# nexus-rl/dfd-starter

Hardware: AMD Instinct MI355X
Metric: env steps/sec (whole node) + sec/FD-grad-step, 4096 antithetic perturbations (higher is better)
Workload: dtype f32; 1 GPU; BASELINE config 3: HalfCheetah-shaped synthetic env (obs 17, act 6), MujocoPolicy(17,6) P=6092, 4096 antithetic perturbations per GPU (2048 directions x +/-), T=1000 fixed-length episodes, full FD step (rollout + weights + gradient + DSGD); perturbations_per_gpu=4096, envs_per_perturbation=1, global_perturbations=4096, episode_len=1000, n_params=6092, parallelism=dp1

## Files before the change

### dfd-starter_amd/csrc/fdr_dpp_gen.h

```cpp
#pragma once

namespace fdr {

__device__ __forceinline__ void dpp_dot_32x1(float& a0, float X0, float X1, const float* w) {
  asm volatile(
      "s_nop 1\n\t"
      "v_mul_f32_dpp %0, %1, %3 row_newbcast:0 row_mask:0xf bank_mask:0xf\n\t"
      "v_fmac_f32_dpp %0, %2, %19 row_newbcast:0 row_mask:0xf bank_mask:0xf\n\t"
      "v_fmac_f32_dpp %0, %1, %4 row_newbcast:1 row_mask:0xf bank_mask:0xf\n\t"
      "v_fmac_f32_dpp %0, %2, %20 row_newbcast:1 row_mask:0xf bank_mask:0xf\n\t"
      "v_fmac_f32_dpp %0, %1, %5 row_newbcast:2 row_mask:0xf bank_mask:0xf\n\t"
      "v_fmac_f32_dpp %0, %2, %21 row_newbcast:2 row_mask:0xf bank_mask:0xf\n\t"
      "v_fmac_f32_dpp %0, %1, %6 row_newbcast:3 row_mask:0xf bank_mask:0xf\n\t"
      "v_fmac_f32_dpp %0, %2, %22 row_newbcast:3 row_mask:0xf bank_mask:0xf\n\t"
      "v_fmac_f32_dpp %0, %1, %7 row_newbcast:4 row_mask:0xf bank_mask:0xf\n\t"
      "v_fmac_f32_dpp %0, %2, %23 row_newbcast:4 row_mask:0xf bank_mask:0xf\n\t"
      "v_fmac_f32_dpp %0, %1, %8 row_newbcast:5 row_mask:0xf bank_mask:0xf\n\t"
      "v_fmac_f32_dpp %0, %2, %24 row_newbcast:5 row_mask:0xf bank_mask:0xf\n\t"
      "v_fmac_f32_dpp %0, %1, %9 row_newbcast:6 row_mask:0xf bank_mask:0xf\n\t"
      "v_fmac_f32_dpp %0, %2, %25 row_newbcast:6 row_mask:0xf bank_mask:0xf\n\t"
      "v_fmac_f32_dpp %0, %1, %10 row_newbcast:7 row_mask:0xf bank_mask:0xf\n\t"
      "v_fmac_f32_dpp %0, %2, %26 row_newbcast:7 row_mask:0xf bank_mask:0xf\n\t"
      "v_fmac_f32_dpp %0, %1, %11 row_newbcast:8 row_mask:0xf bank_mask:0xf\n\t"
      "v_fmac_f32_dpp %0, %2, %27 row_newbcast:8 row_mask:0xf bank_mask:0xf\n\t"
      "v_fmac_f32_dpp %0, %1, %12 row_newbcast:9 row_mask:0xf bank_mask:0xf\n\t"
      "v_fmac_f32_dpp %0, %2, %28 row_newbcast:9 row_mask:0xf bank_mask:0xf\n\t"
      "v_fmac_f32_dpp %0, %1, %13 row_newbcast:10 row_mask:0xf bank_mask:0xf\n\t"
      "v_fmac_f32_dpp %0, %2, %29 row_newbcast:10 row_mask:0xf bank_mask:0xf\n\t"
      "v_fmac_f32_dpp %0, %1, %14 row_newbcast:11 row_mask:0xf bank_mask:0xf\n\t"
      "v_fmac_f32_dpp %0, %2, %30 row_newbcast:11 row_mask:0xf bank_mask:0xf\n\t"
      "v_fmac_f32_dpp %0, %1, %15 row_newbcast:12 row_mask:0xf bank_mask:0xf\n\t"
      "v_fmac_f32_dpp %0, %2, %31 row_newbcast:12 row_mask:0xf bank_mask:0xf\n\t"
      "v_fmac_f32_dpp %0, %1, %16 row_newbcast:13 row_mask:0xf bank_mask:0xf\n\t"
      "v_fmac_f32_dpp %0, %2, %32 row_newbcast:13 row_mask:0xf bank_mask:0xf\n\t"
      "v_fmac_f32_dpp %0, %1, %17 row_newbcast:14 row_mask:0xf bank_mask:0xf\n\t"
      "v_fmac_f32_dpp %0, %2, %33 row_newbcast:14 row_mask:0xf bank_mask:0xf\n\t"
      "v_fmac_f32_dpp %0, %1, %18 row_newbcast:15 row_mask:0xf bank_mask:0xf\n\t"
      "v_fmac_f32_dpp %0, %2, %34 row_newbcast:15 row_mask:0xf bank_mask:0xf\n\t"
      : "=&v"(a0)
      : "v"(X0), "v"(X1), "v"(w[0]), "v"(w[1]), "v"(w[2]), "v"(w[3]), "v"(w[4]), "v"(w[5]), "v"(w[6]), "v"(w[7]), "v"(w[8]), "v"(w[9]), "v"(w[10]), "v"(w[11]), "v"(w[12]), "v"(w[13]), "v"(w[14]), "v"(w[15]), "v"(w[16]), "v"(w[17]), "v"(w[18]), "v"(w[19]), "v"(w[20]), "v"(w[21]), "v"(w[22]), "v"(w[23]), "v"(w[24]), "v"(w[25]), "v"(w[26]), "v"(w[27]), "v"(w[28]), "v"(w[29]), "v"(w[30]), "v"(w[31]));
}
__device__ __forceinline__ void dpp_dot_16x4(float& a0, float& a1, float& a2, float& a3, float X0, const float* w) {
  asm volatile(
      "s_nop 1\n\t"
      "v_mul_f32_dpp %0, %4, %5 row_newbcast:0 row_mask:0xf bank_mask:0xf\n\t"
      "v_mul_f32_dpp %1, %4, %6 row_newbcast:1 row_mask:0xf bank_mask:0xf\n\t"
      "v_mul_f32_dpp %2, %4, %7 row_newbcast:2 row_mask:0xf bank_mask:0xf\n\t"
      "v_mul_f32_dpp %3, %4, %8 row_newbcast:3 row_mask:0xf bank_mask:0xf\n\t"
      "v_fmac_f32_dpp %0, %4, %9 row_newbcast:4 row_mask:0xf bank_mask:0xf\n\t"
      "v_fmac_f32_dpp %1, %4, %10 row_newbcast:5 row_mask:0xf bank_mask:0xf\n\t"
      "v_fmac_f32_dpp %2, %4, %11 row_newbcast:6 row_mask:0xf bank_mask:0xf\n\t"
      "v_fmac_f32_dpp %3, %4, %12 row_newbcast:7 row_mask:0xf bank_mask:0xf\n\t"
      "v_fmac_f32_dpp %0, %4, %13 row_newbcast:8 row_mask:0xf bank_mask:0xf\n\t"
      "v_fmac_f32_dpp %1, %4, %14 row_newbcast:9 row_mask:0xf bank_mask:0xf\n\t"
      "v_fmac_f32_dpp %2, %4, %15 row_newbcast:10 row_mask:0xf bank_mask:0xf\n\t"
      "v_fmac_f32_dpp %3, %4, %16 row_newbcast:11 row_mask:0xf bank_mask:0xf\n\t"
      "v_fmac_f32_dpp %0, %4, %17 row_newbcast:12 row_mask:0xf bank_mask:0xf\n\t"
      "v_fmac_f32_dpp %1, %4, %18 row_newbcast:13 row_mask:0xf bank_mask:0xf\n\t"
      "v_fmac_f32_dpp %2, %4, %19 row_newbcast:14 row_mask:0xf bank_mask:0xf\n\t"
      "v_fmac_f32_dpp %3, %4, %20 row_newbcast:15 row_mask:0xf bank_mask:0xf\n\t"
      : "=&v"(a0), "=&v"(a1), "=&v"(a2), "=&v"(a3)
      : "v"(X0), "v"(w[0]), "v"(w[1]), "v"(w[2]), "v"(w[3]), "v"(w[4]), "v"(w[5]), "v"(w[6]), "v"(w[7]), "v"(w[8]), "v"(w[9]), "v"(w[10]), "v"(w[11]), "v"(w[12]), "v"(w[13]), "v"(w[14]), "v"(w[15]));
}
__device__ __forceinline__ void dpp_fma_tail1(float& a0, float X0, const float* w) {
  asm volatile(
      "s_nop 1\n\t"
      "v_fmac_f32_dpp %0, %1, %2 row_newbcast:0 row_mask:0xf bank_mask:0xf\n\t"
      : "+v"(a0)
      : "v"(X0), "v"(w[0]));
}
__device__ __forceinline__ void dpp_fma_tail2(float& a0, float X0, const float* w) {
  asm volatile(
      "s_nop 1\n\t"
      "v_fmac_f32_dpp %0, %1, %2 row_newbcast:0 row_mask:0xf bank_mask:0xf\n\t"
// ... 166 lines not shown
      "v_fmac_f32_dpp %0, %1, %7 row_newbcast:5 row_mask:0xf bank_mask:0xf\n\t"
      "v_fmac_f32_dpp %0, %1, %8 row_newbcast:6 row_mask:0xf bank_mask:0xf\n\t"
      "v_fmac_f32_dpp %0, %1, %9 row_newbcast:7 row_mask:0xf bank_mask:0xf\n\t"
      "v_fmac_f32_dpp %0, %1, %10 row_newbcast:8 row_mask:0xf bank_mask:0xf\n\t"
      "v_fmac_f32_dpp %0, %1, %11 row_newbcast:9 row_mask:0xf bank_mask:0xf\n\t"
      "v_fmac_f32_dpp %0, %1, %12 row_newbcast:10 row_mask:0xf bank_mask:0xf\n\t"
      "v_fmac_f32_dpp %0, %1, %13 row_newbcast:11 row_mask:0xf bank_mask:0xf\n\t"
      "v_fmac_f32_dpp %0, %1, %14 row_newbcast:12 row_mask:0xf bank_mask:0xf\n\t"
      "v_fmac_f32_dpp %0, %1, %15 row_newbcast:13 row_mask:0xf bank_mask:0xf\n\t"
      : "+v"(a0)
      : "v"(X0), "v"(w[0]), "v"(w[1]), "v"(w[2]), "v"(w[3]), "v"(w[4]), "v"(w[5]), "v"(w[6]), "v"(w[7]), "v"(w[8]), "v"(w[9]), "v"(w[10]), "v"(w[11]), "v"(w[12]), "v"(w[13]));
}
__device__ __forceinline__ void dpp_fma_tail15(float& a0, float X0, const float* w) {
  asm volatile(
      "s_nop 1\n\t"
      "v_fmac_f32_dpp %0, %1, %2 row_newbcast:0 row_mask:0xf bank_mask:0xf\n\t"
      "v_fmac_f32_dpp %0, %1, %3 row_newbcast:1 row_mask:0xf bank_mask:0xf\n\t"
      "v_fmac_f32_dpp %0, %1, %4 row_newbcast:2 row_mask:0xf bank_mask:0xf\n\t"
      "v_fmac_f32_dpp %0, %1, %5 row_newbcast:3 row_mask:0xf bank_mask:0xf\n\t"
      "v_fmac_f32_dpp %0, %1, %6 row_newbcast:4 row_mask:0xf bank_mask:0xf\n\t"
      "v_fmac_f32_dpp %0, %1, %7 row_newbcast:5 row_mask:0xf bank_mask:0xf\n\t"
      "v_fmac_f32_dpp %0, %1, %8 row_newbcast:6 row_mask:0xf bank_mask:0xf\n\t"
      "v_fmac_f32_dpp %0, %1, %9 row_newbcast:7 row_mask:0xf bank_mask:0xf\n\t"
      "v_fmac_f32_dpp %0, %1, %10 row_newbcast:8 row_mask:0xf bank_mask:0xf\n\t"
      "v_fmac_f32_dpp %0, %1, %11 row_newbcast:9 row_mask:0xf bank_mask:0xf\n\t"
      "v_fmac_f32_dpp %0, %1, %12 row_newbcast:10 row_mask:0xf bank_mask:0xf\n\t"
      "v_fmac_f32_dpp %0, %1, %13 row_newbcast:11 row_mask:0xf bank_mask:0xf\n\t"
      "v_fmac_f32_dpp %0, %1, %14 row_newbcast:12 row_mask:0xf bank_mask:0xf\n\t"
      "v_fmac_f32_dpp %0, %1, %15 row_newbcast:13 row_mask:0xf bank_mask:0xf\n\t"
      "v_fmac_f32_dpp %0, %1, %16 row_newbcast:14 row_mask:0xf bank_mask:0xf\n\t"
      : "+v"(a0)
      : "v"(X0), "v"(w[0]), "v"(w[1]), "v"(w[2]), "v"(w[3]), "v"(w[4]), "v"(w[5]), "v"(w[6]), "v"(w[7]), "v"(w[8]), "v"(w[9]), "v"(w[10]), "v"(w[11]), "v"(w[12]), "v"(w[13]), "v"(w[14]));
}
}
```

### dfd-starter_amd/csrc/fdr_mlp_pair.h

```cpp
#pragma once
#include "fdr_mlp.h"

namespace fdr {

constexpr int kPairWaves = 2;

__device__ __forceinline__ f2 tanh2_pre(f2 t) {
  const f2 d = f2{__builtin_amdgcn_exp2f(t.x), __builtin_amdgcn_exp2f(t.y)} + f2{1.f, 1.f};
  return pk_fma(f2{-2.f, -2.f}, f2{__builtin_amdgcn_rcpf(d.x), __builtin_amdgcn_rcpf(d.y)}, f2{1.f, 1.f});
}
__device__ __forceinline__ f2 tanh2_fast(f2 x) {
  return tanh2_pre(x * f2{kTanhScale, kTanhScale});
}
constexpr float kPreScale = kTanhScale;
template <bool kPre>
__device__ __forceinline__ f2 tanh2_act(f2 z) {
  if constexpr (kPre) return tanh2_pre(z);
  else return tanh2_fast(z);
}

template <int NIN, int NA, bool DISC>
struct MlpPair {
  using L = Layout<NIN, NA, DISC>;
  static constexpr int NOUT = L::NOUT;
  static constexpr int NX = round4(NIN);
  static_assert(NX <= 32, "pair kernel: policy input wider than 32");
  static constexpr bool kBiasCol = NIN < NX;
  static constexpr bool kW1Lds = NIN > 8;
  static constexpr bool kPre = !DISC;
  static constexpr float kWS = kPre ? kTanhScale : 1.f;
  static constexpr int kW1Chunks = kW1Lds ? NX / 4 : 0;
  static constexpr int kTileF4 = (2 * kW1Chunks + 8) * kWave;
  f2 w1a[kW1Lds ? 1 : NX / 2], w1b[kW1Lds ? 1 : NX / 2];
  float b1a, b1b;
  const float4* tile;
  f2 w2[64];
  float b2a, b2b, b3;
  float a0, c0, a1a, c1a, a1b, c1b, a2a, c2a, a2b, c2b;

  __host__ __device__ static constexpr int head_unit(int rho, int k, int e) {
    return 32 * rho + 8 * (k >> 2) + 4 * e + (k & 3);
  }

// ... 97 lines not shown
      fold(L::BN1W, L::BN1B, NIN, ua, a1a, c1a);
      fold(L::BN1W, L::BN1B, NIN, ub, a1b, c1b);
      fold(L::BN2W, L::BN2B, NIN + kHidden, u2a, a2a, c2a);
      fold(L::BN2W, L::BN2B, NIN + kHidden, u2b, a2b, c2b);
    }
  }

  __device__ __forceinline__ float input_transform(float x) const {
    if constexpr (DISC) {
      return fmaf(x, a0, c0);
    } else {
      return x;
    }
  }

  __device__ __forceinline__ float act1(float z, float av, float cv) const {
    if constexpr (DISC) {
      return fmaf(fmaxf(z, 0.f), av, cv);
    } else {
      return tanh_act<kPre>(z);
    }
  }

  static constexpr bool kTail = kW1Lds && kBiasCol && NX - NIN == 3;
  static constexpr int NQ = kTail ? NX / 4 - 1 : NX / 4;
  static constexpr bool kPk = kW1Lds && kBiasCol;
  static constexpr int kPkPairs = (NIN + 2) / 2;
  struct L1Rows {
    float4 wa[kW1Lds && !kPk ? NQ : 1], wb[kW1Lds && !kPk ? NQ : 1], m[NQ];
    float2 ta, tb;
    float tm;
    float4 wp[kPk ? kPkPairs : 1];
  };
  __device__ __forceinline__ void l1_prefetch(L1Rows& r, const float* mrow) const {
    const float4* m4 = reinterpret_cast<const float4*>(mrow);
#pragma unroll
    for (int q = 0; q < NQ; ++q) {
      if constexpr (kW1Lds && !kPk) {
        r.wa[q] = tile[q * kWave];
        r.wb[q] = tile[(kW1Chunks + q) * kWave];
      }
      r.m[q] = m4[q];
    }
    if constexpr (kPk) {
#pragma unroll
      for (int j = 0; j < kPkPairs; ++j) r.wp[j] = tile[j * kWave];
      if constexpr (kTail) r.tm = mrow[4 * NQ];
    } else if constexpr (kTail) {
      r.ta = *reinterpret_cast<const float2*>(&tile[NQ * kWave]);
      r.tb = *reinterpret_cast<const float2*>(&tile[(kW1Chunks + NQ) * kWave]);
      r.tm = mrow[4 * NQ];
    }
  }

  struct SIn {
    float4 v[NQ];
    float t;
  };
  template <bool kSameInput, class Fill>
  __device__ __forceinline__ f2 layer1_env(const float* xs, const float* ss, const L1Rows& rows, SIn& sin,
                                           Fill&& fill) const {
    const float4* x4 = reinterpret_cast<const float4*>(xs);
    const float4* s4 = reinterpret_cast<const float4*>(ss);
    SIn xin;
#pragma unroll
    for (int q = 0; q < NQ; ++q) {
      xin.v[q] = x4[q];
      sin.v[q] = kSameInput ? xin.v[q] : s4[q];
    }
    xin.t = kTail ? xs[4 * NQ] : 0.f;
    sin.t = kSameInput ? xin.t : (kTail ? ss[4 * NQ] : 0.f);
    fill();
    __builtin_amdgcn_sched_barrier(0);
    return layer1_q(xin, rows);
  }
  __device__ __forceinline__ float env_ms(const SIn& sin, const L1Rows& rows) const {
    f2 am0 = {0.f, 0.f}, am1 = {0.f, 0.f};
#pragma unroll
    for (int q = 0; q < NQ; ++q) {
      const float4 sv = sin.v[q], mv = rows.m[q];
      am0 = pk_fma(f2{mv.x, mv.y}, f2{sv.x, sv.y}, am0);
      am1 = pk_fma(f2{mv.z, mv.w}, f2{sv.z, sv.w}, am1);
    }
    if constexpr (kTail) am1.x = fmaf(rows.tm, sin.t, am1.x);
    const f2 am = am0 + am1;
    return am.x + am.y;
// ... 40 lines not shown
        return f2{act1(h.x, a1a, c1a), act1(h.y, a1b, c1b)};
      } else {
        return tanh2_act<kPre>(h);
      }
    }
#pragma unroll
    for (int q = 0; q < NQ; ++q) {
      const float4 xv = xq(q);
      float4 wa, wb;
      if constexpr (kW1Lds) {
        wa = rows.wa[q];
        wb = rows.wb[q];
      } else {
        wa = float4{w1a[2 * q].x, w1a[2 * q].y, w1a[2 * q + 1].x, w1a[2 * q + 1].y};
        wb = float4{w1b[2 * q].x, w1b[2 * q].y, w1b[2 * q + 1].x, w1b[2 * q + 1].y};
      }
      aa0 = pk_fma(f2{wa.x, wa.y}, f2{xv.x, xv.y}, aa0);
      ab0 = pk_fma(f2{wb.x, wb.y}, f2{xv.x, xv.y}, ab0);
      aa1 = pk_fma(f2{wa.z, wa.w}, f2{xv.z, xv.w}, aa1);
      ab1 = pk_fma(f2{wb.z, wb.w}, f2{xv.z, xv.w}, ab1);
    }
    if constexpr (kTail) {
      aa1 = pk_fma(f2{rows.ta.x, rows.ta.y}, f2{xt, 1.f}, aa1);
      ab1 = pk_fma(f2{rows.tb.x, rows.tb.y}, f2{xt, 1.f}, ab1);
    }
    const f2 ha = aa0 + aa1, hb = ab0 + ab1;
    if constexpr (DISC) {
      return f2{act1(ha.x + ha.y, a1a, c1a), act1(hb.x + hb.y, a1b, c1b)};
    } else {
      return tanh2_act<kPre>(f2{ha.x + ha.y, hb.x + hb.y});
    }
  }

  template <class Mark>
  __device__ __forceinline__ float layers23(f2 h1, float* h1s, int t, Mark&& mark) const {
    const int c4 = t & 3;
    float x[16];
    reinterpret_cast<f2*>(h1s)[t] = h1;
    __builtin_amdgcn_s_setprio(0);
    wave_lds_sync();
    lds_bcast<16>(h1s + 16 * c4, x);
    float w3[32];
#pragma unroll
    for (int m = 0; m < 8; ++m) {
      const float4 w = tile[(2 * kW1Chunks + m) * kWave];
      w3[4 * m] = w.x;
      w3[4 * m + 1] = w.y;
      w3[4 * m + 2] = w.z;
      w3[4 * m + 3] = w.w;
    }
    f2 acc[4];
#pragma unroll
    for (int p = 0; p < 4; ++p)
      acc[p] = pk_fma(w2[p * 16], f2{x[0], x[0]}, (kPre && p == 0) ? f2{b2a, b2b} : f2{0.f, 0.f});
    {
      f2 xp[8];
#pragma unroll
      for (int j = 0; j < 8; ++j) xp[j] = f2{x[2 * j], x[2 * j + 1]};
#define FDR_L2_HI "op_sel:[0,1,0] op_sel_hi:[1,1,1]"
#define FDR_L2_LO "op_sel_hi:[1,0,1]"
      asm(
          "v_pk_fma_f32 %0, %4, %64, %0 " FDR_L2_HI "\n"
          "v_pk_fma_f32 %1, %5, %64, %1 " FDR_L2_HI "\n"
          "v_pk_fma_f32 %2, %6, %64, %2 " FDR_L2_HI "\n"
          "v_pk_fma_f32 %3, %7, %64, %3 " FDR_L2_HI "\n"
          "v_pk_fma_f32 %0, %8, %65, %0 " FDR_L2_LO "\n"
          "v_pk_fma_f32 %1, %9, %65, %1 " FDR_L2_LO "\n"
          "v_pk_fma_f32 %2, %10, %65, %2 " FDR_L2_LO "\n"
// ... 40 lines not shown
          "v_pk_fma_f32 %3, %51, %70, %3 " FDR_L2_LO "\n"
          "v_pk_fma_f32 %0, %52, %70, %0 " FDR_L2_HI "\n"
          "v_pk_fma_f32 %1, %53, %70, %1 " FDR_L2_HI "\n"
          "v_pk_fma_f32 %2, %54, %70, %2 " FDR_L2_HI "\n"
          "v_pk_fma_f32 %3, %55, %70, %3 " FDR_L2_HI "\n"
          "v_pk_fma_f32 %0, %56, %71, %0 " FDR_L2_LO "\n"
          "v_pk_fma_f32 %1, %57, %71, %1 " FDR_L2_LO "\n"
          "v_pk_fma_f32 %2, %58, %71, %2 " FDR_L2_LO "\n"
          "v_pk_fma_f32 %3, %59, %71, %3 " FDR_L2_LO "\n"
          "v_pk_fma_f32 %3, %63, %71, %3 " FDR_L2_HI "\n"
          "v_pk_fma_f32 %2, %62, %71, %2 " FDR_L2_HI "\n"
          "v_pk_fma_f32 %0, %60, %71, %0 " FDR_L2_HI "\n"
          "v_pk_fma_f32 %1, %61, %71, %1 " FDR_L2_HI "\n"
          : "+v"(acc[0]), "+v"(acc[1]), "+v"(acc[2]), "+v"(acc[3])
          : "v"(w2[1]), "v"(w2[17]), "v"(w2[33]), "v"(w2[49]),
            "v"(w2[2]), "v"(w2[18]), "v"(w2[34]), "v"(w2[50]),
            "v"(w2[3]), "v"(w2[19]), "v"(w2[35]), "v"(w2[51]),
            "v"(w2[4]), "v"(w2[20]), "v"(w2[36]), "v"(w2[52]),
            "v"(w2[5]), "v"(w2[21]), "v"(w2[37]), "v"(w2[53]),
            "v"(w2[6]), "v"(w2[22]), "v"(w2[38]), "v"(w2[54]),
            "v"(w2[7]), "v"(w2[23]), "v"(w2[39]), "v"(w2[55]),
            "v"(w2[8]), "v"(w2[24]), "v"(w2[40]), "v"(w2[56]),
            "v"(w2[9]), "v"(w2[25]), "v"(w2[41]), "v"(w2[57]),
            "v"(w2[10]), "v"(w2[26]), "v"(w2[42]), "v"(w2[58]),
            "v"(w2[11]), "v"(w2[27]), "v"(w2[43]), "v"(w2[59]),
            "v"(w2[12]), "v"(w2[28]), "v"(w2[44]), "v"(w2[60]),
            "v"(w2[13]), "v"(w2[29]), "v"(w2[45]), "v"(w2[61]),
            "v"(w2[14]), "v"(w2[30]), "v"(w2[46]), "v"(w2[62]),
            "v"(w2[15]), "v"(w2[31]), "v"(w2[47]), "v"(w2[63]),
            "v"(xp[0]), "v"(xp[1]), "v"(xp[2]), "v"(xp[3]), "v"(xp[4]), "v"(xp[5]), "v"(xp[6]), "v"(xp[7]));
#undef FDR_L2_LO
#undef FDR_L2_HI
    }
    f2 zs;
    __builtin_amdgcn_s_setprio(1);
    {
      float o0, o1, o2, o3;
      asm volatile(
          "v_add_f32_dpp %2, %10, %6 quad_perm:[2,3,0,1] row_mask:0xf bank_mask:0xf bound_ctrl:1\n\t"
          "v_add_f32_dpp %3, %11, %7 quad_perm:[2,3,0,1] row_mask:0xf bank_mask:0xf bound_ctrl:1\n\t"
          "v_add_f32_dpp %0, %8, %4 quad_perm:[2,3,0,1] row_mask:0xf bank_mask:0xf bound_ctrl:1\n\t"
          "v_add_f32_dpp %1, %9, %5 quad_perm:[2,3,0,1] row_mask:0xf bank_mask:0xf bound_ctrl:1\n\t"
          "v_add_f32_dpp %0, %2, %0 quad_perm:[1,0,3,2] row_mask:0xf bank_mask:0xf bound_ctrl:1\n\t"
          "v_add_f32_dpp %1, %3, %1 quad_perm:[1,0,3,2] row_mask:0xf bank_mask:0xf bound_ctrl:1\n\t"
          : "=&v"(o0), "=&v"(o1), "=&v"(o2), "=&v"(o3)
          : "v"(acc[0].x), "v"(acc[0].y), "v"(acc[1].x), "v"(acc[1].y), "v"(acc[2].x), "v"(acc[2].y), "v"(acc[3].x),
            "v"(acc[3].y));
      zs = f2{o0, o1};
    }
    const float za = kPre ? zs.x : zs.x + b2a;
    const float zb = kPre ? zs.y : zs.y + b2b;
    mark(1, za);
    float h2a, h2b;
    if constexpr (DISC) {
      h2a = fmaf(fmaxf(za, 0.f), a2a, c2a);
      h2b = fmaf(fmaxf(zb, 0.f), a2b, c2b);
    } else {
      const f2 h2 = tanh2_act<kPre>(f2{za, zb});
      h2a = h2.x;
      h2b = h2.y;
    }
    float u;
    dpp_dot_32x1(u, h2a, h2b, w3);
    float v = u;
    permlane16_swap(u, v);
    const float out = (u + v) + b3;
    mark(2, out);
    return out;
  }

  template <bool kAll = false, bool kFast = false>
  __device__ __forceinline__ float softmax(float logit, int t) const {
    const bool valid = (t & 15) < NOUT;
    const float v = valid ? logit : -FLT_MAX;
    const float mx = row16_max_n<NOUT>(v);
    if constexpr (kFast) {
      const float e = valid ? __builtin_amdgcn_exp2f((v - mx) * 1.44269504088896341f) : 0.f;
      return e * __builtin_amdgcn_rcpf(row16_sum_n<NOUT>(e));
    } else {
      const float e = valid ? expf(v - mx) : 0.f;
      return e / row16_sum_n<NOUT>(e);
    }
  }
};

struct alignas(16) PairScratch {
  float h1[2][kHidden];
  float x[2][32];
};

template <int K>
__device__ __forceinline__ float row_bcast(float v) {
  return __builtin_bit_cast(float, __builtin_amdgcn_mov_dpp(__builtin_bit_cast(int, v), 0x150 + K, 0xF, 0xF, false));
}

template <int N, int... I>
__device__ __forceinline__ void row_bcast_all(float v, float (&out)[N], std::integer_sequence<int, I...>) {
  ((out[I] = row_bcast<I>(v)), ...);
}

}
```

### dfd-starter_amd/csrc/fdr_rollout_pair.hip

```cpp
#include <algorithm>

#include "fdr_mlp_pair.h"

namespace fdr {

#ifndef FDR_STEP_LOOP_PAD
#define FDR_STEP_LOOP_PAD 15
#endif
#if FDR_STEP_LOOP_PAD >= 0
#define FDR_STR2(x) #x
#define FDR_STR(x) FDR_STR2(x)
#define FDR_STEP_LOOP_PLACED asm volatile(".p2align 6\n\t.rept " FDR_STR(FDR_STEP_LOOP_PAD) "\n\ts_nop 0\n\t.endr");
#else
#define FDR_STEP_LOOP_PLACED
#endif

template <int NIN, int NA, bool DISC, int FEAT>
__global__ __launch_bounds__(64 * kPairWaves, 2) void rollout_pair_kernel(RolloutArgs a) {
  using Lane = MlpPair<NIN, NA, DISC>;
  constexpr int NX = Lane::NX;
  constexpr int NMK = NX + round4(NA);
  constexpr int MKS = NMK % 8 == 0 ? NMK + 4 : NMK;
  __shared__ float4 env4[NIN * MKS / 4];
  __shared__ float4 wtile[kPairWaves * Lane::kTileF4];
// ... 20 lines not shown
#pragma unroll
    for (int m = 16; m >= 1; m >>= 1) n2 += __shfl_xor(n2, m, kWave);
    asm volatile("" : "+v"(n2));
    if (t == 0 && active && a.norm2) a.norm2[lane] = n2;
  }

  const int ji = t < NIN ? t : NIN - 1;
  constexpr bool norm_obs = (FEAT & kFeatObsNorm) != 0;
  const float om = norm_obs ? a.obs_mean[ji] : 0.f;
  const float osd = norm_obs ? a.obs_std[ji] : 1.f;
  auto policy_input = [&](float s) {
    float x = s;
    if (norm_obs) x = fminf(fmaxf((s - om) / osd, -10.f), 10.f);
    return pl.input_transform(x);
  };
  float s = a.s0[ji];
  const int T = a.T;
  const uint64_t key = a.key;
  const uint64_t ulane = (uint64_t)(a.lanes.lane_offset + lane);
  double racc = 0.0;
  float eacc = 0.f;
  const int o = t & 15;
  constexpr int kDrawsPerStep = DISC ? 1 : NA;
  constexpr int kStepsPerBatch = 32 / kDrawsPerStep;
  constexpr bool kTerm = (FEAT & kFeatTerm) != 0;
  bool alive0 = true, alive1 = true;
  int n0 = T, n1 = T;
  auto alive_me = [&]() { return hh ? alive1 : alive0; };
  float rbuf = 0.f;
  const int zbase = 4 * (32 * hh + (DISC ? 0 : (o < NA ? o : 0)));
  auto* sc = &scratch[wv];
  [[maybe_unused]] float* xs = sc->x[hh];
  float* h1s = sc->h1[hh];
  const float* mrow = envMK + ji * MKS;
  constexpr bool kSame = !DISC && !norm_obs;
  typename Lane::L1Rows l1rows;
  pl.l1_prefetch(l1rows, mrow);
  float kr[DISC ? 1 : NA];
#pragma unroll
  for (int m = 0; m < (DISC ? 1 : NA); ++m) kr[m] = mrow[NX + m];
  int tb = 0;
#ifdef FDR_PHASE_STAMPS
  uint64_t ph_acc[5] = {0, 0, 0, 0, 0};
  uint64_t ph_last = 0;
  auto mark = [&](int k, float dep) {
    uint64_t now;
    asm volatile("s_memtime %0\n\ts_waitcnt lgkmcnt(0)" : "=s"(now) : "v"(dep));
    if (k >= 0) ph_acc[k] += now - ph_last;
    ph_last = now;
  };
#else
  auto mark = [](int, float) {};
#endif
  auto draw = [&](int st) {
    const int ds = t / kDrawsPerStep, dk = t % kDrawsPerStep;
    const uint64_t hsh = hash_ctr(key, ulane, (uint64_t)(st + ds), (uint64_t)dk);
    rbuf = DISC ? uniform24(hsh) : normal_bm(hsh);
  };
  int dctr = ((t / kDrawsPerStep) << 4) | (t % kDrawsPerStep);
  uint64_t dz = 0;
  float du1 = 0.f, du2 = 0.f;
  auto draw_part = [&](int k, int st) {
    if (k == 0) {
      asm volatile("" : "+v"(dctr)::"memory");
      dz = mix64_a(key + (((uint64_t)ulane << 32) | (uint64_t)((st << 4) + dctr)) * 0x9E3779B97F4A7C15ull);
    } else if (k == 1) {
      asm volatile("" : "+v"(dz)::"memory");
      dz = mix64_b(dz);
    } else if (k == 2) {
      asm volatile("" : "+v"(dz)::"memory");
      const uint64_t hsh = mix64_c(dz);
      du1 = bm_u1(hsh);
      du2 = bm_u2(hsh);
    } else if (k == 3) {
      asm volatile("" : "+v"(du1)::"memory");
      du1 = bm_radius(du1);
    } else if (k == 4) {
      asm volatile("" : "+v"(du1), "+v"(du2)::"memory");
      rbuf = bm_normal(du1, du2);
    }
  };
  auto step = [&](int st, int tb, auto&& fill) {
    const float zt = __builtin_bit_cast(
        float, __builtin_amdgcn_ds_bpermute(zbase + 4 * kDrawsPerStep * tb, __builtin_bit_cast(int, rbuf)));
    if constexpr (FEAT & kFeatStates) {
      if (t < NIN && active && (!kTerm || alive_me())) a.states[((int64_t)lane * T + st) * NIN + t] = s;
    }
    float pre = 0.f;
    xs[t] = t < NIN ? policy_input(s) : (t == NIN ? 1.f : 0.f);
    if constexpr (!kSame) h1s[t] = t < NIN ? s : 0.f;
    wave_lds_sync();
    typename Lane::SIn sin;
    const f2 h1 = pl.template layer1_env<kSame>(xs, h1s, l1rows, sin, fill);
    pre = pl.env_ms(sin, l1rows);

    mark(0, h1.x);
    const float y = pl.layers23(h1, h1s, t, mark);
    pl.l1_prefetch(l1rows, mrow);
    if constexpr (DISC) {
      const float p = det ? pl.softmax(y, t) : pl.template softmax<false, true>(y, t);
      float pv[NA];
      row_bcast_all(p, pv, std::make_integer_sequence<int, NA>{});
      float tot = 0.f;
#pragma unroll
      for (int i = 0; i < NA; ++i) tot += pv[i];
      int act_d = 0;
      if (det) {
        float best = pv[0];
#pragma unroll
        for (int i = 1; i < NA; ++i) {
          act_d = pv[i] > best ? i : act_d;
          best = fmaxf(best, pv[i]);
        }
      } else {
        const float target = zt * tot;
        float cs = 0.f;
#pragma unroll
        for (int i = 0; i < NA - 1; ++i) {
          cs += pv[i];
          act_d += cs <= target ? 1 : 0;
        }
      }
      eacc -= (o < NA && (!kTerm || alive_me())) ? disc_entropy_term(p, tot) : 0.f;
      pre += mrow[NX + act_d];
    } else {
      const float th = tanh_act<Lane::kPre>(y);
      const float sd = std_from_tanh(dpp_mov<kDppRowShl + NA>(th));
      if constexpr (kTerm)
        eacc += alive_me() ? __builtin_amdgcn_logf(sd) : 0.f;
      else
        eacc += __builtin_amdgcn_logf(sd);
      const float act_c = det ? th : gauss_action(th, sd, zt);
      mark(3, act_c);
      dpp_tail<NA>(pre, act_c, kr);
    }
    s = tanh_pre(pre);
    mark(4, s);
    if constexpr (kTerm) {
      racc += alive_me() ? (double)s : 0.0;
      const bool d0 = fabsf(readlane_f(s, a.done_dim)) > a.done_thr;
      const bool d1 = fabsf(readlane_f(s, 32 + a.done_dim)) > a.done_thr;
      if (alive0 && d0) {
        alive0 = false;
        n0 = st + 1;
      }
      if (alive1 && d1) {
        alive1 = false;
        n1 = st + 1;
      }
      return !alive0 && !alive1;
    } else {
      racc += (double)s;
      return false;
    }
  };
  if constexpr (!DISC) {
    [&] {
      int st = 0;
      draw(0);
      FDR_STEP_LOOP_PLACED
      for (; st + kStepsPerBatch <= T; st += kStepsPerBatch) {
        asm volatile("" ::: "memory");
        mark(-1, s);
#pragma unroll
        for (int k = 0; k < kStepsPerBatch; ++k) {
          if (k) {
            asm volatile("" ::: "memory");
            mark(-1, s);
          }
          constexpr int kLast = kStepsPerBatch - 1;
          static_assert(kLast >= 4, "draw_part: five parts need a batch of five steps");
          const int part = k == kLast ? 4 : (k < 4 ? k : -1);
          if (step(st + k, k, [&] { draw_part(part, st + kStepsPerBatch); })) return;
        }
      }
      if (st < T) {
        for (int k = 0; st + k < T; ++k) {
          asm volatile("" ::: "memory");
          mark(-1, s);
          if (step(st + k, k, [] {})) return;
        }
      }
    }();
  } else {
    for (int st = 0; st < T; ++st) {
      asm volatile("" ::: "memory");
      mark(-1, s);
      if (!det && tb == 0) draw(st);
      if (step(st, tb, [] {})) break;
      tb = tb + 1 == kStepsPerBatch ? 0 : tb + 1;
    }
  }
// ... 45 lines not shown
```

### dfd-starter_amd/csrc/fdr_wave.h

```cpp
#pragma once
#include <hip/hip_runtime.h>

#include "fdr_dpp_gen.h"

namespace fdr {

__device__ __forceinline__ void permlane32_swap(float& a, float& b) {
  asm volatile("s_nop 1\n\tv_permlane32_swap_b32 %0, %1" : "+v"(a), "+v"(b));
}
__device__ __forceinline__ void permlane16_swap(float& a, float& b) {
  asm volatile("s_nop 1\n\tv_permlane16_swap_b32 %0, %1" : "+v"(a), "+v"(b));
}

__device__ __forceinline__ float row_allreduce_sum(float v) {
  float a = v, b = v;
  permlane32_swap(a, b);
  float s = a + b;
  float c = s, d = s;
  permlane16_swap(c, d);
  return c + d;
}

template <int N>
__device__ __forceinline__ void dpp_tail(float& acc, float X, const float* w) {
  static_assert(N >= 0 && N < 16, "tail of 0..15 inputs");
  if constexpr (N == 1) dpp_fma_tail1(acc, X, w);
  if constexpr (N == 2) dpp_fma_tail2(acc, X, w);
  if constexpr (N == 3) dpp_fma_tail3(acc, X, w);
  if constexpr (N == 4) dpp_fma_tail4(acc, X, w);
  if constexpr (N == 5) dpp_fma_tail5(acc, X, w);
  if constexpr (N == 6) dpp_fma_tail6(acc, X, w);
  if constexpr (N == 7) dpp_fma_tail7(acc, X, w);
  if constexpr (N == 8) dpp_fma_tail8(acc, X, w);
  if constexpr (N == 9) dpp_fma_tail9(acc, X, w);
  if constexpr (N == 10) dpp_fma_tail10(acc, X, w);
  if constexpr (N == 11) dpp_fma_tail11(acc, X, w);
  if constexpr (N == 12) dpp_fma_tail12(acc, X, w);
  if constexpr (N == 13) dpp_fma_tail13(acc, X, w);
  if constexpr (N == 14) dpp_fma_tail14(acc, X, w);
  if constexpr (N == 15) dpp_fma_tail15(acc, X, w);
}

__device__ __forceinline__ float dot_row16(float v, const float* w) {
  float a0, a1, a2, a3;
  dpp_dot_16x4(a0, a1, a2, a3, v, w);
  return (a0 + a2) + (a1 + a3);
}

template <int CTRL>
__device__ __forceinline__ float dpp_mov(float v) {
  return __builtin_bit_cast(float, __builtin_amdgcn_mov_dpp(__builtin_bit_cast(int, v), CTRL, 0xF, 0xF, true));
}
constexpr int kDppQuadXor1 = 0xB1;
constexpr int kDppQuadXor2 = 0x4E;
constexpr int kDppHalfMirror = 0x141;
constexpr int kDppMirror = 0x140;
constexpr int kDppRowShl = 0x100;
constexpr int kDppRowRor = 0x120;

__device__ __forceinline__ float row16_max(float v) {
  v = fmaxf(v, dpp_mov<kDppQuadXor1>(v));
  v = fmaxf(v, dpp_mov<kDppQuadXor2>(v));
  v = fmaxf(v, dpp_mov<kDppHalfMirror>(v));
  v = fmaxf(v, dpp_mov<kDppMirror>(v));
  return v;
}
__device__ __forceinline__ float row16_sum(float v) {
  v += dpp_mov<kDppQuadXor1>(v);
  v += dpp_mov<kDppQuadXor2>(v);
  v += dpp_mov<kDppHalfMirror>(v);
  v += dpp_mov<kDppMirror>(v);
  return v;
}
// ... 30 lines not shown
```

Baseline: 4.800 billion env steps/s.

## Fill DPP/transcendental hazard pads with split layer-1 prefetch loads in pair rollout

Splits the next-step layer-1 row prefetch into ranged chunks and places them inside the wait slots of the layer-2 tanh, layer-3 DPP dot, permlane swap and action tanh, replacing explicit s_nop pads. The layer-2 reduction and tanh are fused into one asm block, and the entropy log is folded into the action tail asm. Other changes: the constant x padding is written once outside the step loop, the deterministic draw becomes a branchless zero noise, and an s0 dependency hint is added. All of this is enabled by default through macros. The scheduling relies on sched_barrier fences and on removing s_nop hazard padding, which risks a DPP hazard violation or a worse schedule if the fill chunks do not cover the required latency.

```diff
diff --git a/dfd-starter_amd/csrc/fdr_dpp_gen.h b/dfd-starter_amd/csrc/fdr_dpp_gen.h
--- a/dfd-starter_amd/csrc/fdr_dpp_gen.h
+++ b/dfd-starter_amd/csrc/fdr_dpp_gen.h
@@ -40,6 +40,44 @@
       : "=&v"(a0)
       : "v"(X0), "v"(X1), "v"(w[0]), "v"(w[1]), "v"(w[2]), "v"(w[3]), "v"(w[4]), "v"(w[5]), "v"(w[6]), "v"(w[7]), "v"(w[8]), "v"(w[9]), "v"(w[10]), "v"(w[11]), "v"(w[12]), "v"(w[13]), "v"(w[14]), "v"(w[15]), "v"(w[16]), "v"(w[17]), "v"(w[18]), "v"(w[19]), "v"(w[20]), "v"(w[21]), "v"(w[22]), "v"(w[23]), "v"(w[24]), "v"(w[25]), "v"(w[26]), "v"(w[27]), "v"(w[28]), "v"(w[29]), "v"(w[30]), "v"(w[31]));
 }
+__device__ __forceinline__ void dpp_dot_32x1_copy(float& a0, float& c0, float X0, float X1, const float* w) {
+  asm volatile(
+      "v_mul_f32_dpp %0, %2, %4 row_newbcast:0 row_mask:0xf bank_mask:0xf\n\t"
+      "v_fmac_f32_dpp %0, %3, %20 row_newbcast:0 row_mask:0xf bank_mask:0xf\n\t"
+      "v_fmac_f32_dpp %0, %2, %5 row_newbcast:1 row_mask:0xf bank_mask:0xf\n\t"
+      "v_fmac_f32_dpp %0, %3, %21 row_newbcast:1 row_mask:0xf bank_mask:0xf\n\t"
+      "v_fmac_f32_dpp %0, %2, %6 row_newbcast:2 row_mask:0xf bank_mask:0xf\n\t"
+      "v_fmac_f32_dpp %0, %3, %22 row_newbcast:2 row_mask:0xf bank_mask:0xf\n\t"
+      "v_fmac_f32_dpp %0, %2, %7 row_newbcast:3 row_mask:0xf bank_mask:0xf\n\t"
+      "v_fmac_f32_dpp %0, %3, %23 row_newbcast:3 row_mask:0xf bank_mask:0xf\n\t"
+      "v_fmac_f32_dpp %0, %2, %8 row_newbcast:4 row_mask:0xf bank_mask:0xf\n\t"
+      "v_fmac_f32_dpp %0, %3, %24 row_newbcast:4 row_mask:0xf bank_mask:0xf\n\t"
+      "v_fmac_f32_dpp %0, %2, %9 row_newbcast:5 row_mask:0xf bank_mask:0xf\n\t"
+      "v_fmac_f32_dpp %0, %3, %25 row_newbcast:5 row_mask:0xf bank_mask:0xf\n\t"
+      "v_fmac_f32_dpp %0, %2, %10 row_newbcast:6 row_mask:0xf bank_mask:0xf\n\t"
+      "v_fmac_f32_dpp %0, %3, %26 row_newbcast:6 row_mask:0xf bank_mask:0xf\n\t"
+      "v_fmac_f32_dpp %0, %2, %11 row_newbcast:7 row_mask:0xf bank_mask:0xf\n\t"
+      "v_fmac_f32_dpp %0, %3, %27 row_newbcast:7 row_mask:0xf bank_mask:0xf\n\t"
+      "v_fmac_f32_dpp %0, %2, %12 row_newbcast:8 row_mask:0xf bank_mask:0xf\n\t"
+      "v_fmac_f32_dpp %0, %3, %28 row_newbcast:8 row_mask:0xf bank_mask:0xf\n\t"
+      "v_fmac_f32_dpp %0, %2, %13 row_newbcast:9 row_mask:0xf bank_mask:0xf\n\t"
+      "v_fmac_f32_dpp %0, %3, %29 row_newbcast:9 row_mask:0xf bank_mask:0xf\n\t"
+      "v_fmac_f32_dpp %0, %2, %14 row_newbcast:10 row_mask:0xf bank_mask:0xf\n\t"
+      "v_fmac_f32_dpp %0, %3, %30 row_newbcast:10 row_mask:0xf bank_mask:0xf\n\t"
+      "v_fmac_f32_dpp %0, %2, %15 row_newbcast:11 row_mask:0xf bank_mask:0xf\n\t"
+      "v_fmac_f32_dpp %0, %3, %31 row_newbcast:11 row_mask:0xf bank_mask:0xf\n\t"
+      "v_fmac_f32_dpp %0, %2, %16 row_newbcast:12 row_mask:0xf bank_mask:0xf\n\t"
+      "v_fmac_f32_dpp %0, %3, %32 row_newbcast:12 row_mask:0xf bank_mask:0xf\n\t"
+      "v_fmac_f32_dpp %0, %2, %17 row_newbcast:13 row_mask:0xf bank_mask:0xf\n\t"
+      "v_fmac_f32_dpp %0, %3, %33 row_newbcast:13 row_mask:0xf bank_mask:0xf\n\t"
+      "v_fmac_f32_dpp %0, %2, %18 row_newbcast:14 row_mask:0xf bank_mask:0xf\n\t"
+      "v_fmac_f32_dpp %0, %3, %34 row_newbcast:14 row_mask:0xf bank_mask:0xf\n\t"
+      "v_fmac_f32_dpp %0, %2, %19 row_newbcast:15 row_mask:0xf bank_mask:0xf\n\t"
+      "v_fmac_f32_dpp %0, %3, %35 row_newbcast:15 row_mask:0xf bank_mask:0xf\n\t"
+      "v_mov_b32 %1, %0\n\t"
+      : "=&v"(a0), "=&v"(c0)
+      : "v"(X0), "v"(X1), "v"(w[0]), "v"(w[1]), "v"(w[2]), "v"(w[3]), "v"(w[4]), "v"(w[5]), "v"(w[6]), "v"(w[7]), "v"(w[8]), "v"(w[9]), "v"(w[10]), "v"(w[11]), "v"(w[12]), "v"(w[13]), "v"(w[14]), "v"(w[15]), "v"(w[16]), "v"(w[17]), "v"(w[18]), "v"(w[19]), "v"(w[20]), "v"(w[21]), "v"(w[22]), "v"(w[23]), "v"(w[24]), "v"(w[25]), "v"(w[26]), "v"(w[27]), "v"(w[28]), "v"(w[29]), "v"(w[30]), "v"(w[31]));
+}
 __device__ __forceinline__ void dpp_dot_16x4(float& a0, float& a1, float& a2, float& a3, float X0, const float* w) {
   asm volatile(
       "s_nop 1\n\t"
@@ -272,4 +310,33 @@
       : "+v"(a0)
       : "v"(X0), "v"(w[0]), "v"(w[1]), "v"(w[2]), "v"(w[3]), "v"(w[4]), "v"(w[5]), "v"(w[6]), "v"(w[7]), "v"(w[8]), "v"(w[9]), "v"(w[10]), "v"(w[11]), "v"(w[12]), "v"(w[13]), "v"(w[14]));
 }
-}
+__device__ __forceinline__ void dpp_fma_tail2_log(float& a0, float& lg, float X0, float Y, const float* w) {
+  asm volatile(
+      "v_log_f32 %1, %3\n\t"
+      "v_fmac_f32_dpp %0, %2, %4 row_newbcast:0 row_mask:0xf bank_mask:0xf\n\t"
+      "v_fmac_f32_dpp %0, %2, %5 row_newbcast:1 row_mask:0xf bank_mask:0xf\n\t"
+      : "+v"(a0), "=&v"(lg)
+      : "v"(X0), "v"(Y), "v"(w[0]), "v"(w[1]));
+}
+__device__ __forceinline__ void dpp_fma_tail3_log(float& a0, float& lg, float X0, float Y, const float* w) {
+  asm volatile(
+      "v_log_f32 %1, %3\n\t"
+      "v_fmac_f32_dpp %0, %2, %4 row_newbcast:0 row_mask:0xf bank_mask:0xf\n\t"
+      "v_fmac_f32_dpp %0, %2, %5 row_newbcast:1 row_mask:0xf bank_mask:0xf\n\t"
+      "v_fmac_f32_dpp %0, %2, %6 row_newbcast:2 row_mask:0xf bank_mask:0xf\n\t"
+      : "+v"(a0), "=&v"(lg)
+      : "v"(X0), "v"(Y), "v"(w[0]), "v"(w[1]), "v"(w[2]));
+}
+__device__ __forceinline__ void dpp_fma_tail6_log(float& a0, float& lg, float X0, float Y, const float* w) {
+  asm volatile(
+      "v_log_f32 %1, %3\n\t"
+      "v_fmac_f32_dpp %0, %2, %4 row_newbcast:0 row_mask:0xf bank_mask:0xf\n\t"
+      "v_fmac_f32_dpp %0, %2, %5 row_newbcast:1 row_mask:0xf bank_mask:0xf\n\t"
+      "v_fmac_f32_dpp %0, %2, %6 row_newbcast:2 row_mask:0xf bank_mask:0xf\n\t"
+      "v_fmac_f32_dpp %0, %2, %7 row_newbcast:3 row_mask:0xf bank_mask:0xf\n\t"
+      "v_fmac_f32_dpp %0, %2, %8 row_newbcast:4 row_mask:0xf bank_mask:0xf\n\t"
+      "v_fmac_f32_dpp %0, %2, %9 row_newbcast:5 row_mask:0xf bank_mask:0xf\n\t"
+      : "+v"(a0), "=&v"(lg)
+      : "v"(X0), "v"(Y), "v"(w[0]), "v"(w[1]), "v"(w[2]), "v"(w[3]), "v"(w[4]), "v"(w[5]));
+}
+}
diff --git a/dfd-starter_amd/csrc/fdr_mlp_pair.h b/dfd-starter_amd/csrc/fdr_mlp_pair.h
--- a/dfd-starter_amd/csrc/fdr_mlp_pair.h
+++ b/dfd-starter_amd/csrc/fdr_mlp_pair.h
@@ -4,11 +4,41 @@
 namespace fdr {
 
 constexpr int kPairWaves = 2;
+
+#ifndef FDR_PAIR_FILL_PADS
+#define FDR_PAIR_FILL_PADS 1
+#endif
+#ifndef FDR_PAIR_TANH8
+#define FDR_PAIR_TANH8 1
+#endif
+#ifndef FDR_PAIR_DET_DRAW
+#define FDR_PAIR_DET_DRAW 1
+#endif
+#ifndef FDR_PAIR_X_TAIL
+#define FDR_PAIR_X_TAIL 1
+#endif
+#ifndef FDR_PAIR_S0_WAIT
+#define FDR_PAIR_S0_WAIT 1
+#endif
 
 __device__ __forceinline__ f2 tanh2_pre(f2 t) {
   const f2 d = f2{__builtin_amdgcn_exp2f(t.x), __builtin_amdgcn_exp2f(t.y)} + f2{1.f, 1.f};
   return pk_fma(f2{-2.f, -2.f}, f2{__builtin_amdgcn_rcpf(d.x), __builtin_amdgcn_rcpf(d.y)}, f2{1.f, 1.f});
 }
+template <class FX, class FY>
+__device__ __forceinline__ float tanh_pre_fill(float t, FX&& fx, FY&& fy) {
+  const float e = __builtin_amdgcn_exp2f(t);
+  __builtin_amdgcn_sched_barrier(0);
+  fx();
+  __builtin_amdgcn_sched_barrier(0);
+  const float r = __builtin_amdgcn_rcpf(1.0f + e);
+  __builtin_amdgcn_sched_barrier(0);
+  fy();
+  __builtin_amdgcn_sched_barrier(0);
+  return 1.0f - 2.0f * r;
+}
+template <int V>
+using ic = std::integral_constant<int, V>;
 __device__ __forceinline__ f2 tanh2_fast(f2 x) {
   return tanh2_pre(x * f2{kTanhScale, kTanhScale});
 }
@@ -172,26 +202,46 @@
     float tm;
     float4 wp[kPk ? kPkPairs : 1];
   };
+  static constexpr int kRowReads = NQ + (kPk ? kPkPairs : kW1Lds ? 2 * NQ : 0) + (kTail ? (kPk ? 1 : 3) : 0);
+  template <int LO = 0, int HI = kRowReads>
   __device__ __forceinline__ void l1_prefetch(L1Rows& r, const float* mrow) const {
     const float4* m4 = reinterpret_cast<const float4*>(mrow);
-#pragma unroll
-    for (int q = 0; q < NQ; ++q) {
-      if constexpr (kW1Lds && !kPk) {
-        r.wa[q] = tile[q * kWave];
-        r.wb[q] = tile[(kW1Chunks + q) * kWave];
-      }
-      r.m[q] = m4[q];
-    }
+    int i = 0;
+    auto on = [&] {
+      const bool y = i >= LO && i < HI;
+      ++i;
+      return y;
+    };
+#pragma unroll
+    for (int q = 0; q < NQ; ++q)
+      if (on()) r.m[q] = m4[q];
     if constexpr (kPk) {
 #pragma unroll
-      for (int j = 0; j < kPkPairs; ++j) r.wp[j] = tile[j * kWave];
-      if constexpr (kTail) r.tm = mrow[4 * NQ];
-    } else if constexpr (kTail) {
-      r.ta = *reinterpret_cast<const float2*>(&tile[NQ * kWave]);
-      r.tb = *reinterpret_cast<const float2*>(&tile[(kW1Chunks + NQ) * kWave]);
-      r.tm = mrow[4 * NQ];
-    }
-  }
+      for (int j = 0; j < kPkPairs; ++j)
+        if (on()) r.wp[j] = tile[j * kWave];
+      if constexpr (kTail)
+        if (on()) r.tm = mrow[4 * NQ];
+    } else if constexpr (kW1Lds) {
+#pragma unroll
+      for (int q = 0; q < NQ; ++q) {
+        if (on()) r.wa[q] = tile[q * kWave];
+        if (on()) r.wb[q] = tile[(kW1Chunks + q) * kWave];
+      }
+      if constexpr (kTail) {
+        if (on()) r.ta = *reinterpret_cast<const float2*>(&tile[NQ * kWave]);
+        if (on()) r.tb = *reinterpret_cast<const float2*>(&tile[(kW1Chunks + NQ) * kWave]);
+        if (on()) r.tm = mrow[4 * NQ];
+      }
+    }
+  }
+  static constexpr int kFill =
+      !FDR_PAIR_FILL_PADS || DISC ? 0 : (FDR_PAIR_TANH8 && kRowReads >= 11) ? 2 : kRowReads >= 4 ? 1 : 0;
+  struct FillPlan {
+    static constexpr int N = kRowReads;
+    static constexpr int kHead = kFill ? 1 : 0, kSwap = kFill ? 3 : 0, kSum = kFill == 2 ? 4 : kSwap;
+    static constexpr int kExp = kFill == 2 ? N - 4 : kSum, kRcp = kFill == 2 ? N - 3 : kSum;
+    static constexpr int kMov = kFill ? N - 1 : 0, kAll = kFill ? N : 0;
+  };
 
   struct SIn {
     float4 v[NQ];
@@ -298,8 +348,9 @@
     }
   }
 
-  template <class Mark>
-  __device__ __forceinline__ float layers23(f2 h1, float* h1s, int t, Mark&& mark) const {
+  template <class Mark, class FillA, class FillB, class FillC>
+  __device__ __forceinline__ float layers23(f2 h1, float* h1s, int t, Mark&& mark, FillA&& fill_a, FillB&& fill_b,
+                                            FillC&& fill_c) const {
     const int c4 = t & 3;
     float x[16];
     reinterpret_cast<f2*>(h1s)[t] = h1;
@@ -406,38 +457,80 @@
 #undef FDR_L2_LO
 #undef FDR_L2_HI
     }
-    f2 zs;
+#define FDR_PAIR_RS                                                                              \
+  "v_add_f32_dpp %2, %10, %6 quad_perm:[2,3,0,1] row_mask:0xf bank_mask:0xf bound_ctrl:1\n\t" \
+  "v_add_f32_dpp %3, %11, %7 quad_perm:[2,3,0,1] row_mask:0xf bank_mask:0xf bound_ctrl:1\n\t" \
+  "v_add_f32_dpp %0, %8, %4 quad_perm:[2,3,0,1] row_mask:0xf bank_mask:0xf bound_ctrl:1\n\t"  \
+  "v_add_f32_dpp %1, %9, %5 quad_perm:[2,3,0,1] row_mask:0xf bank_mask:0xf bound_ctrl:1\n\t"  \
+  "v_add_f32_dpp %0, %2, %0 quad_perm:[1,0,3,2] row_mask:0xf bank_mask:0xf bound_ctrl:1\n\t"  \
+  "v_add_f32_dpp %1, %3, %1 quad_perm:[1,0,3,2] row_mask:0xf bank_mask:0xf bound_ctrl:1\n\t"
     __builtin_amdgcn_s_setprio(1);
-    {
-      float o0, o1, o2, o3;
+    float h2a, h2b;
+#ifdef FDR_PHASE_STAMPS
+    constexpr bool kAb = false;
+#else
+    constexpr bool kAb = FDR_PAIR_TANH8 && kPre;
+#endif
+    if constexpr (kAb) {
+      float o2, o3;
       asm volatile(
-          "v_add_f32_dpp %2, %10, %6 quad_perm:[2,3,0,1] row_mask:0xf bank_mask:0xf bound_ctrl:1\n\t"
-          "v_add_f32_dpp %3, %11, %7 quad_perm:[2,3,0,1] row_mask:0xf bank_mask:0xf bound_ctrl:1\n\t"
-          "v_add_f32_dpp %0, %8, %4 quad_perm:[2,3,0,1] row_mask:0xf bank_mask:0xf bound_ctrl:1\n\t"
-          "v_add_f32_dpp %1, %9, %5 quad_perm:[2,3,0,1] row_mask:0xf bank_mask:0xf bound_ctrl:1\n\t"
-          "v_add_f32_dpp %0, %2, %0 quad_perm:[1,0,3,2] row_mask:0xf bank_mask:0xf bound_ctrl:1\n\t"
-          "v_add_f32_dpp %1, %3, %1 quad_perm:[1,0,3,2] row_mask:0xf bank_mask:0xf bound_ctrl:1\n\t"
-          : "=&v"(o0), "=&v"(o1), "=&v"(o2), "=&v"(o3)
+          FDR_PAIR_RS
+          "v_exp_f32 %0, %0\n\t"
+          "v_exp_f32 %1, %1\n\t"
+          "v_add_f32 %0, 1.0, %0\n\t"
+          "v_add_f32 %1, 1.0, %1\n\t"
+          "v_rcp_f32 %0, %0\n\t"
+          "v_rcp_f32 %1, %1\n\t"
+          "v_fma_f32 %0, %0, -2.0, 1.0\n\t"
+          "v_fma_f32 %1, %1, -2.0, 1.0"
+          : "=&v"(h2a), "=&v"(h2b), "=&v"(o2), "=&v"(o3)
           : "v"(acc[0].x), "v"(acc[0].y), "v"(acc[1].x), "v"(acc[1].y), "v"(acc[2].x), "v"(acc[2].y), "v"(acc[3].x),
             "v"(acc[3].y));
-      zs = f2{o0, o1};
-    }
-    const float za = kPre ? zs.x : zs.x + b2a;
-    const float zb = kPre ? zs.y : zs.y + b2b;
-    mark(1, za);
-    float h2a, h2b;
-    if constexpr (DISC) {
-      h2a = fmaf(fmaxf(za, 0.f), a2a, c2a);
-      h2b = fmaf(fmaxf(zb, 0.f), a2b, c2b);
-    } else {
-      const f2 h2 = tanh2_act<kPre>(f2{za, zb});
-      h2a = h2.x;
-      h2b = h2.y;
-    }
-    float u;
-    dpp_dot_32x1(u, h2a, h2b, w3);
-    float v = u;
-    permlane16_swap(u, v);
+    } else {
+      f2 zs;
+      {
+        float o0, o1, o2, o3;
+        asm volatile(
+            FDR_PAIR_RS
+            : "=&v"(o0), "=&v"(o1), "=&v"(o2), "=&v"(o3)
+            : "v"(acc[0].x), "v"(acc[0].y), "v"(acc[1].x), "v"(acc[1].y), "v"(acc[2].x), "v"(acc[2].y), "v"(acc[3].x),
+              "v"(acc[3].y));
+        zs = f2{o0, o1};
+      }
+      const float za = kPre ? zs.x : zs.x + b2a;
+      const float zb = kPre ? zs.y : zs.y + b2b;
+      mark(1, za);
+      if constexpr (DISC) {
+        h2a = fmaf(fmaxf(za, 0.f), a2a, c2a);
+        h2b = fmaf(fmaxf(zb, 0.f), a2b, c2b);
+      } else {
+        const f2 h2 = tanh2_act<kPre>(f2{za, zb});
+        h2a = h2.x;
+        h2b = h2.y;
+      }
+    }
+#undef FDR_PAIR_RS
+    float u, v;
+    if constexpr (kFill != 0) {
+      __builtin_amdgcn_sched_barrier(0);
+      fill_a();
+      __builtin_amdgcn_sched_barrier(0);
+      if constexpr (!kAb) asm volatile("s_nop 0");
+      dpp_dot_32x1_copy(u, v, h2a, h2b, w3);
+      __builtin_amdgcn_sched_barrier(0);
+      fill_b();
+      __builtin_amdgcn_sched_barrier(0);
+      permlane16_swap_nopad(u, v);
+      if constexpr (kFill == 2) {
+        __builtin_amdgcn_sched_barrier(0);
+        fill_c();
+        __builtin_amdgcn_sched_barrier(0);
+      }
+    } else {
+      dpp_dot_32x1(u, h2a, h2b, w3);
+      v = u;
+      permlane16_swap(u, v);
+    }
     const float out = (u + v) + b3;
     mark(2, out);
     return out;
@@ -461,6 +554,7 @@
 struct alignas(16) PairScratch {
   float h1[2][kHidden];
   float x[2][32];
+  float dead[4];
 };
 
 template <int K>
diff --git a/dfd-starter_amd/csrc/fdr_rollout_pair.hip b/dfd-starter_amd/csrc/fdr_rollout_pair.hip
--- a/dfd-starter_amd/csrc/fdr_rollout_pair.hip
+++ b/dfd-starter_amd/csrc/fdr_rollout_pair.hip
@@ -76,6 +76,11 @@
   auto* sc = &scratch[wv];
   [[maybe_unused]] float* xs = sc->x[hh];
   float* h1s = sc->h1[hh];
+#if FDR_PAIR_X_TAIL
+  float* xw = t < NIN ? xs + t : sc->dead + hh;
+  if (t >= NIN) xs[t] = t == NIN ? 1.f : 0.f;
+  wave_lds_sync();
+#endif
   const float* mrow = envMK + ji * MKS;
   constexpr bool kSame = !DISC && !norm_obs;
   typename Lane::L1Rows l1rows;
@@ -100,6 +105,7 @@
     const int ds = t / kDrawsPerStep, dk = t % kDrawsPerStep;
     const uint64_t hsh = hash_ctr(key, ulane, (uint64_t)(st + ds), (uint64_t)dk);
     rbuf = DISC ? uniform24(hsh) : normal_bm(hsh);
+    if constexpr (!DISC && FDR_PAIR_DET_DRAW) rbuf = det ? -0.0f : rbuf;
   };
   int dctr = ((t / kDrawsPerStep) << 4) | (t % kDrawsPerStep);
   uint64_t dz = 0;
@@ -122,6 +128,7 @@
     } else if (k == 4) {
       asm volatile("" : "+v"(du1), "+v"(du2)::"memory");
       rbuf = bm_normal(du1, du2);
+      if constexpr (FDR_PAIR_DET_DRAW) rbuf = det ? -0.0f : rbuf;
     }
   };
   auto step = [&](int st, int tb, auto&& fill) {
@@ -131,7 +138,11 @@
       if (t < NIN && active && (!kTerm || alive_me())) a.states[((int64_t)lane * T + st) * NIN + t] = s;
     }
     float pre = 0.f;
+#if FDR_PAIR_X_TAIL
+    *xw = policy_input(s);
+#else
     xs[t] = t < NIN ? policy_input(s) : (t == NIN ? 1.f : 0.f);
+#endif
     if constexpr (!kSame) h1s[t] = t < NIN ? s : 0.f;
     wave_lds_sync();
     typename Lane::SIn sin;
@@ -139,8 +150,14 @@
     pre = pl.env_ms(sin, l1rows);
 
     mark(0, h1.x);
-    const float y = pl.layers23(h1, h1s, t, mark);
-    pl.l1_prefetch(l1rows, mrow);
+    using F = typename Lane::FillPlan;
+    auto rows = [&](auto lo, auto hi) {
+      pl.template l1_prefetch<decltype(lo)::value, decltype(hi)::value>(l1rows, mrow);
+    };
+    const float y = pl.layers23(
+        h1, h1s, t, mark, [&] { rows(ic<0>{}, ic<F::kHead>{}); }, [&] { rows(ic<F::kHead>{}, ic<F::kSwap>{}); },
+        [&] { rows(ic<F::kSwap>{}, ic<F::kSum>{}); });
+    if constexpr (Lane::kFill == 0) pl.l1_prefetch(l1rows, mrow);
     if constexpr (DISC) {
       const float p = det ? pl.softmax(y, t) : pl.template softmax<false, true>(y, t);
       float pv[NA];
@@ -168,15 +185,37 @@
       eacc -= (o < NA && (!kTerm || alive_me())) ? disc_entropy_term(p, tot) : 0.f;
       pre += mrow[NX + act_d];
     } else {
-      const float th = tanh_act<Lane::kPre>(y);
+      float th;
+      if constexpr (Lane::kFill == 2) {
+        th = tanh_pre_fill(y, [&] { rows(ic<F::kSum>{}, ic<F::kExp>{}); }, [&] { rows(ic<F::kExp>{}, ic<F::kRcp>{}); });
+        __builtin_amdgcn_sched_barrier(0);
+        rows(ic<F::kRcp>{}, ic<F::kMov>{});
+        __builtin_amdgcn_sched_barrier(0);
+      } else {
+        rows(ic<F::kSum>{}, ic<F::kMov>{});
+        th = tanh_act<Lane::kPre>(y);
+      }
       const float sd = std_from_tanh(dpp_mov<kDppRowShl + NA>(th));
-      if constexpr (kTerm)
-        eacc += alive_me() ? __builtin_amdgcn_logf(sd) : 0.f;
-      else
-        eacc += __builtin_amdgcn_logf(sd);
-      const float act_c = det ? th : gauss_action(th, sd, zt);
+      const float act_c = FDR_PAIR_DET_DRAW ? gauss_action(th, sd, zt) : (det ? th : gauss_action(th, sd, zt));
       mark(3, act_c);
-      dpp_tail<NA>(pre, act_c, kr);
+      float lg;
+      auto add_entropy = [&] {
+        if constexpr (kTerm)
+          eacc += alive_me() ? lg : 0.f;
+        else
+          eacc += lg;
+      };
+      if constexpr (Lane::kFill) {
+        __builtin_amdgcn_sched_barrier(0);
+        rows(ic<F::kMov>{}, ic<F::kAll>{});
+        __builtin_amdgcn_sched_barrier(0);
+        dpp_tail_log<NA>(pre, lg, act_c, sd, kr);
+        __builtin_amdgcn_sched_barrier(0);
+      } else {
+        lg = __builtin_amdgcn_logf(sd);
+        dpp_tail<NA>(pre, act_c, kr);
+      }
+      add_entropy();
     }
     s = tanh_pre(pre);
     mark(4, s);
@@ -202,6 +241,9 @@
     [&] {
       int st = 0;
       draw(0);
+#if FDR_PAIR_S0_WAIT
+      asm volatile("" : "+v"(s));
+#endif
       FDR_STEP_LOOP_PLACED
       for (; st + kStepsPerBatch <= T; st += kStepsPerBatch) {
         asm volatile("" ::: "memory");
diff --git a/dfd-starter_amd/csrc/fdr_wave.h b/dfd-starter_amd/csrc/fdr_wave.h
--- a/dfd-starter_amd/csrc/fdr_wave.h
+++ b/dfd-starter_amd/csrc/fdr_wave.h
@@ -10,6 +10,10 @@
 }
 __device__ __forceinline__ void permlane16_swap(float& a, float& b) {
   asm volatile("s_nop 1\n\tv_permlane16_swap_b32 %0, %1" : "+v"(a), "+v"(b));
+}
+
+__device__ __forceinline__ void permlane16_swap_nopad(float& a, float& b) {
+  asm volatile("v_permlane16_swap_b32 %0, %1" : "+v"(a), "+v"(b));
 }
 
 __device__ __forceinline__ float row_allreduce_sum(float v) {
@@ -39,6 +43,14 @@
   if constexpr (N == 13) dpp_fma_tail13(acc, X, w);
   if constexpr (N == 14) dpp_fma_tail14(acc, X, w);
   if constexpr (N == 15) dpp_fma_tail15(acc, X, w);
+}
+
+template <int N>
+__device__ __forceinline__ void dpp_tail_log(float& acc, float& lg, float X, float Y, const float* w) {
+  static_assert(N == 2 || N == 3 || N == 6, "generated for the pair kernel's continuous action widths");
+  if constexpr (N == 2) dpp_fma_tail2_log(acc, lg, X, Y, w);
+  if constexpr (N == 3) dpp_fma_tail3_log(acc, lg, X, Y, w);
+  if constexpr (N == 6) dpp_fma_tail6_log(acc, lg, X, Y, w);
 }
 
 __device__ __forceinline__ float dot_row16(float v, const float* w) {
```

After: 4.844 billion env steps/s, median of 6. No clear change (+0.9%).
